# turlando/flac-py

Measured on AMD Instinct MI355X. Metric: PCM samples/sec encode-analysis, 4608-blk/16-bit mono, 1/2/4/8 MI355X, higher is better.
Workload: dtype i16 in; f64 autocorrelation/Levinson; i32 predictors; 1 GPU; 1e6 synthetic mono 4608-sample int16 blocks, -l 12 -q 5 -r 0,5; units_per_gpu=1000000, units_total=1000000, block=4608, sample_bits=16, max_lpc_order=12, qlp_precision=5, mode=reference, parallelism=dp1 (block shards), open_eighths=0, lpc_pruning=on: candidates proven to lose skipped (sign bound, partial-sum tiers)

## Files before the change

### flac-py_amd/abi.py

```python
import ctypes as C

import numpy as np

ABI_VERSION = 6
MAX_LPC_ORDER = 32
MAX_BLOCK = 65535
MAX_RICE_ORDER = 15
STATS_WORDS = 128
E_INVALID, E_HIP, E_UNSUPPORTED, E_NOMEM = -1, -2, -3, -4


def lpc_rec_words(L: int) -> int:
    return 2 + L + (L * (L + 1)) // 2


STATUS_OK = 0
STATUS_ZERO_DIVISION = 1
STATUS_ASSERTION = 2
STATUS_VALUE_ERROR = 3
STATUS_OVERFLOW = 4
STATUS_RESIDUAL_WIDE = 16
STATUS_FRAME_TOO_LARGE = 17
STATUS_EOF = 5
STATUS_VERIFY = 18
# ... 369 lines not shown
                                          C.c_int32, C.c_void_p, C.c_void_p, C.c_void_p, C.c_int64, C.c_int64,
                                          C.POINTER(InfoResult)]),
    "flacmi_stream_stats": (C.c_int, [C.c_void_p, C.c_void_p, C.c_int64, C.c_int32, C.c_int32,
                                      C.c_int64, C.c_void_p, C.c_void_p]),
    "flacmi_comm_available": (C.c_int, []),
    "flacmi_unit_stride": (C.c_int64, [C.c_int32, C.c_int32]),
    "flacmi_comm_id": (C.c_int, [C.c_void_p]),
    "flacmi_comm_init": (C.c_int, [C.c_void_p, C.c_int, C.c_int, C.c_void_p, C.POINTER(C.c_void_p)]),
    "flacmi_allreduce_stats": (C.c_int, [C.c_void_p, C.c_void_p, C.c_void_p]),
    "flacmi_comm_destroy": (C.c_int, [C.c_void_p]),
    "flacmi_synth_device": (C.c_int, [C.c_void_p, C.c_void_p, C.c_int32, C.c_int32, C.c_int64,
                                      C.c_int64, C.c_int64, C.c_int32, C.c_uint64, C.c_void_p]),
    "flacmi_synth_mix_device": (C.c_int, [C.c_void_p, C.c_void_p, C.c_int32, C.c_int32, C.c_int64,
                                          C.c_int64, C.c_int64, C.c_int32, C.c_uint64, C.c_int32, C.c_void_p]),
    "flacmi_device_alloc": (C.c_void_p, [C.c_void_p, C.c_size_t]),
    "flacmi_device_free": (C.c_int, [C.c_void_p, C.c_void_p]),
    "flacmi_memcpy_h2d": (C.c_int, [C.c_void_p, C.c_void_p, C.c_void_p, C.c_size_t]),
    "flacmi_memcpy_d2h": (C.c_int, [C.c_void_p, C.c_void_p, C.c_void_p, C.c_size_t]),
    "flacmi_synchronize": (C.c_int, [C.c_void_p]),
    "flacmi_last_timing": (C.c_int, [C.c_void_p, C.POINTER(C.c_float), C.c_int]),
    "flacmi_timing_reset": (C.c_int, [C.c_void_p]),
    "flacmi_set_knob": (C.c_int, [C.c_char_p, C.c_int32]),
    "flacmi_get_knob": (C.c_int, [C.c_char_p, C.POINTER(C.c_int32)]),
    "flacmi_host_pypow2": (C.c_double, [C.c_double, C.POINTER(C.c_int32)]),
    "flacmi_host_floor_log2": (C.c_int32, [C.c_double]),
    "flacmi_device_selftest": (C.c_int, [C.c_void_p, C.c_int32, C.c_void_p, C.c_void_p, C.c_void_p,
                                         C.c_int64]),
    "flacmi_device_lpc_from_acf": (C.c_int, [C.c_void_p, C.c_void_p, C.c_int64, C.c_int32, C.c_int32,
                                             C.c_void_p]),
}
```

### flac-py_amd/csrc/flacmi_host.cpp

```cpp
#include <dlfcn.h>
#include <hip/hip_runtime.h>

#include <algorithm>
#include <atomic>
#include <cerrno>
#include <chrono>
#include <cmath>
#include <cstdarg>
#include <cstdio>
#include <cstdlib>
#include <cstring>
#include <map>
#include <mutex>
#include <string>
#include <vector>

#include "../../include/flacmi.h"
#include "flacmi_kernels.h"
#include "pymath.h"
#include "device_common.h"

using namespace flacmi;

static double (*volatile libm_cos)(double) = cos;
// ... 102 lines not shown
struct flacmi_ctx {
    int device = 0;
    hipStream_t stream = nullptr;
    double* d_log2thr = nullptr;
    int32_t* d_sintab = nullptr;
    std::map<int, double*> windows;
    std::map<int, std::pair<int, int>> window_one;
    std::map<int, uint16_t*> chunk_weights;
    DevBuf bound;
    DevBuf rec, retry, h_samples, h_meta, h_params, h_residual, h_acf, h_fs, h_ls, h_recs;
    uint16_t* d_crc = nullptr;
    DevBuf scan, h_offsets, h_status, h_frames, dec, slow;
    DevBuf h_subkind;
    DevBuf h_wasted;
    DevBuf h_side, h_choice;
    DevBuf idx, sd_data, sd_table, sd_meta, sd_rows, sd_pcm;
    DevBuf si_frames, si_subs, si_parts;
    int64_t frames_bytes = 0;
    static constexpr int kRing = 64;
    static constexpr int kMaxChunks = 8;
    hipEvent_t ev[kRing][3 + 2 * kMaxChunks] = {};
    int nchunks[kRing] = {};
    hipEvent_t lpc_done[kMaxChunks] = {};
    int ncalls = 0;
    struct EncState* enc = nullptr;
};
static void enc_free(struct EncState* es);
static int enc_streams(flacmi_ctx* ctx);
static hipStream_t enc_side(flacmi_ctx* ctx);

static int ensure_buf(DevBuf& b, size_t bytes) {
    if (b.bytes >= bytes && b.p) return 0;
    if (b.p) HIP_TRY(hipFree(b.p));
    b.p = nullptr;
    b.bytes = 0;
    size_t want = bytes + bytes / 8 + 4096;
    HIP_TRY(hipMalloc(&b.p, want));
    b.bytes = want;
    return 0;
}

static int64_t row_pitch(int64_t n, int64_t sample_bytes) {
    int64_t bytes = ((n * sample_bytes + 15) / 16) * 16;
    if (bytes % 4096 == 0) bytes += 128;
    return bytes / sample_bytes;
}

static int set_device(flacmi_ctx* ctx) {
    if (!ctx) return fail(FLACMI_E_INVALID, "null context");
    HIP_TRY(hipSetDevice(ctx->device));
    return 0;
}

namespace {
struct KnobDef {
    const char* name;
    int dflt;
};
constexpr KnobDef kKnobs[kKnobCount] = {{"FLACMI_OVERLAP", -1}, {"FLACMI_MF8_GRID", 0}, {"FLACMI_STREAM_GENERIC", 0}, {"FLACMI_DECODE_GENERIC", 0},
                                        {"FLACMI_PACK_GENERIC", 0}, {"FLACMI_DECODE_LPC", 1}, {"FLACMI_ENERGY_BOUND", 1}, {"FLACMI_INFO_GRID", 0},
                                        {"FLACMI_RICE_GRID", 0}};
std::atomic<int> g_knob[kKnobCount];
std::once_flag g_knob_once;
void knobs_init() {
    std::call_once(g_knob_once, [] {
        for (int i = 0; i < kKnobCount; ++i) {
            const char* e = getenv(kKnobs[i].name);
            g_knob[i].store(e && e[0] ? atoi(e) : kKnobs[i].dflt);
        }
    });
}
int knob_index(const char* name) {
    if (!name) return -1;
    for (int i = 0; i < kKnobCount; ++i)
        if (strcmp(name, kKnobs[i].name) == 0) return i;
    return -1;
}
}

int flacmi::knob(Knob k) {
    knobs_init();
    return g_knob[k].load(std::memory_order_relaxed);
}

extern "C" {

int flacmi_set_knob(const char* name, int32_t value) {
    const int i = knob_index(name);
    if (i < 0) return fail(FLACMI_E_INVALID, "unknown knob %s", name ? name : "(null)");
    knobs_init();
    g_knob[i].store(value);
    return 0;
}

int flacmi_get_knob(const char* name, int32_t* value) {
    const int i = knob_index(name);
    if (i < 0 || !value) return fail(FLACMI_E_INVALID, "unknown knob %s", name ? name : "(null)");
    *value = knob((Knob)i);
    return 0;
}

int flacmi_abi_version(void) { return FLACMI_ABI_VERSION; }

const char* flacmi_last_error(void) { return g_err.c_str(); }

int flacmi_device_count(void) {
    int n = 0;
    if (hipGetDeviceCount(&n) != hipSuccess) return 0;
    return n;
}

flacmi_ctx* flacmi_create(int device) {
    ensure_tables();
    if (!g_tables_error.empty()) {
        fail(FLACMI_E_UNSUPPORTED, "%s", g_tables_error.c_str());
        return nullptr;
    }
    int ndev = 0;
    if (hipGetDeviceCount(&ndev) != hipSuccess || ndev <= 0) {
        fail(FLACMI_E_HIP, "no HIP device available");
        return nullptr;
    }
    if (device < 0 || device >= ndev) {
        fail(FLACMI_E_INVALID, "device %d out of range (0..%d)", device, ndev - 1);
        return nullptr;
    }
    flacmi_ctx* ctx = new flacmi_ctx();
    ctx->device = device;
    auto bad = [&](hipError_t e, const char* what) {
        fail(FLACMI_E_HIP, "%s: %s", what, hipGetErrorString(e));
        flacmi_destroy(ctx);
        return (flacmi_ctx*)nullptr;
    };
    hipError_t e;
    if ((e = hipSetDevice(device)) != hipSuccess) return bad(e, "hipSetDevice");
    if ((e = hipStreamCreateWithFlags(&ctx->stream, hipStreamNonBlocking)) != hipSuccess) return bad(e, "hipStreamCreate");
    for (auto& slot : ctx->ev)
        for (auto& ev : slot)
            if ((e = hipEventCreate(&ev)) != hipSuccess) return bad(e, "hipEventCreate");
    for (auto& ev : ctx->lpc_done)
        if ((e = hipEventCreateWithFlags(&ev, hipEventDisableTiming)) != hipSuccess) return bad(e, "hipEventCreate");
    if ((e = hipMalloc(&ctx->d_log2thr, sizeof(double) * PYM_LOG2_THR_N)) != hipSuccess) return bad(e, "hipMalloc");
    if ((e = hipMemcpy(ctx->d_log2thr, g_log2thr.data(), sizeof(double) * PYM_LOG2_THR_N, hipMemcpyHostToDevice)) != hipSuccess)
        return bad(e, "hipMemcpy");
    if ((e = hipMalloc(&ctx->d_sintab, sizeof(int32_t) * 4096)) != hipSuccess) return bad(e, "hipMalloc");
    if ((e = hipMemcpy(ctx->d_sintab, g_sintab.data(), sizeof(int32_t) * 4096, hipMemcpyHostToDevice)) != hipSuccess)
        return bad(e, "hipMemcpy");
    const std::vector<uint16_t> crc = crc16_tables();
    if ((e = hipMalloc(&ctx->d_crc, sizeof(uint16_t) * crc.size())) != hipSuccess) return bad(e, "hipMalloc");
    if ((e = hipMemcpy(ctx->d_crc, crc.data(), sizeof(uint16_t) * crc.size(), hipMemcpyHostToDevice)) != hipSuccess)
        return bad(e, "hipMemcpy");
    return ctx;
}

void flacmi_destroy(flacmi_ctx* ctx) {
    if (!ctx) return;
    (void)hipSetDevice(ctx->device);
    (void)hipDeviceSynchronize();
    enc_free(ctx->enc);
    for (auto& kv : ctx->windows) (void)hipFree(kv.second);
    for (auto& kv : ctx->chunk_weights) (void)hipFree(kv.second);
    for (DevBuf* b : {&ctx->bound, &ctx->idx, &ctx->sd_data, &ctx->sd_table, &ctx->sd_meta, &ctx->sd_rows, &ctx->sd_pcm, &ctx->si_frames, &ctx->si_subs, &ctx->si_parts, &ctx->slow, &ctx->dec, &ctx->rec, &ctx->retry, &ctx->h_samples, &ctx->h_meta, &ctx->h_params, &ctx->h_residual, &ctx->h_acf,
                      &ctx->h_fs, &ctx->h_ls, &ctx->h_recs, &ctx->scan, &ctx->h_offsets, &ctx->h_status,
                      &ctx->h_frames, &ctx->h_subkind, &ctx->h_side, &ctx->h_choice, &ctx->h_wasted})
        if (b->p) (void)hipFree(b->p);
    if (ctx->d_log2thr) (void)hipFree(ctx->d_log2thr);
    if (ctx->d_sintab) (void)hipFree(ctx->d_sintab);
    if (ctx->d_crc) (void)hipFree(ctx->d_crc);
    for (auto& slot : ctx->ev)
        for (auto& ev : slot)
            if (ev) (void)hipEventDestroy(ev);
    if (ctx->stream) (void)hipStreamDestroy(ctx->stream);
    for (auto& ev : ctx->lpc_done)
        if (ev) (void)hipEventDestroy(ev);
    delete ctx;
}

}

static void bound_tables(const std::vector<double>& w, int n, double* kappa, std::vector<uint16_t>& cw) {
    for (int k = 1; k <= kBoundLags; ++k) {
        double m = 0.0;
        for (int i = k; i <= n - 2; ++i) m = std::max(m, fabs(w[i] - w[i - k]));
        kappa[k - 1] = m * (1.0 + ldexp(1.0, -50));
    }
    cw.assign((size_t)(n + 7) / 8, 0);
    for (int c = 2; 8 * c < n; ++c) {
        double m = 1.0;
        for (int i = 8 * c; i < 8 * c + 8; ++i) m = std::min(m, i < n - 1 ? w[i] : 0.0);
        cw[c] = (uint16_t)floor(256.0 * m);
    }
}

static int get_window(flacmi_ctx* ctx, int n, double** out, int* one_lo = nullptr, int* one_hi = nullptr,
                      const uint16_t** chunk_weight = nullptr) {
    auto it = ctx->windows.find(n);
    if (it == ctx->windows.end()) {
// ... 165 lines not shown
#ifndef FLACMI_CLASS_LISTS
#define FLACMI_CLASS_LISTS 1
#endif
static int overlap_mode() { return knob(kKnobOverlap); }

static int analyze_device_impl(flacmi_ctx* ctx, const flacmi_batch* b, const flacmi_params* p,
                               const flacmi_outputs* o, hipStream_t s, bool allow_overlap = true) {
    if (int rc = set_device(ctx)) return rc;
    const bool lpc = p->mode == FLACMI_MODE_REFERENCE || p->mode == FLACMI_MODE_LPC_ONLY;
    const int L = lpc ? p->max_lpc_order : 0;
    const int rec_words = FLACMI_LPC_REC_WORDS(L);
    if (lpc) {
        if (int rc = ensure_buf(ctx->rec, sizeof(int32_t) * (size_t)rec_words * (size_t)(b->n_units > 0 ? b->n_units : 1)))
            return rc;
    }
    const int energy = debug_stop() >= 11 ? 0 : knob(kKnobEnergyBound);
    const bool prune_call = p->mode == FLACMI_MODE_REFERENCE && !o->lpc_sums &&
                            !(p->reserved[1] & (FLACMI_FLAG_ALL_CANDIDATES | FLACMI_FLAG_LPC_SIGN | FLACMI_FLAG_SIZE_CHOICE)) && prune_allowed();
    const bool ebound = energy != 0 && prune_call && L >= 1 && L <= 12 && b->sample_bytes == 2 && p->qlp_precision <= 16;
    if (ebound) {
        if (int rc = ensure_buf(ctx->bound, sizeof(uint32_t) * kBoundWords * (size_t)(b->n_units > 0 ? b->n_units : 1))) return rc;
    }
    constexpr int64_t kSubWords = 64 * 16;
    if (int rc = ensure_buf(ctx->retry, sizeof(int64_t) * (size_t)(kSubWords + 2 * b->n_units + 68))) return rc;
    struct Cls {
        int64_t unit0, count;
        int n;
    } cls[2];
    int ncls = 0;
    const int64_t nfull = b->n_units - b->n_tail_units;
    if (b->n_tail_units == 0 || b->tail_len == b->block_len) {
        cls[ncls++] = {0, b->n_units, b->block_len};
    } else {
        if (nfull > 0) cls[ncls++] = {0, nfull, b->block_len};
        cls[ncls++] = {nfull, b->n_tail_units, b->tail_len};
    }
    if (o->acf && !lpc)
        HIP_TRY(hipMemsetAsync(o->acf, 0, sizeof(double) * 33 * b->n_units, s));
    struct Chunk {
        int64_t unit0, count;
        int n;
    } ch[flacmi_ctx::kMaxChunks];
    auto lpc_params_for = [&](int n) {
        LpcArgs a{};
        a.stride = b->unit_stride;
        a.sample_bytes = b->sample_bytes;
        a.n = n;
        a.L = L;
        return a;
    };
    int nch = 0;
    const int ov = lpc ? overlap_mode() : 0;
    const int want = ov > 1 ? ov : 1;
    bool overlap = want > 1 && b->n_units >= 2 * kOverlapMinUnits;
    for (int c = 0; c < ncls; ++c) {
        if (ov < -1 || (ov == -1 && cls[c].count >= 2 * kOverlapMinUnits)) {
            const int64_t R = ov < -1 ? -(int64_t)ov : lpc_units_per_round(lpc_params_for(cls[c].n));
            const int64_t whole = R > 0 ? cls[c].count / R * R : 0, rest = cls[c].count - whole;
            if (whole > 0 && rest > 0 && (ov < -1 || rest >= kOverlapMinUnits) &&
                nch + 2 + (ncls - 1 - c) <= flacmi_ctx::kMaxChunks) {
                ch[nch++] = {cls[c].unit0, whole, cls[c].n};
                ch[nch++] = {cls[c].unit0 + whole, rest, cls[c].n};
                overlap = true;
                continue;
            }
        }
        int64_t k = overlap && ov > 1 ? cls[c].count / kOverlapMinUnits : 1;
        const int left = flacmi_ctx::kMaxChunks - nch - (ncls - 1 - c);
        k = k < 1 ? 1 : k > want ? want : k;
        k = k > left ? left : k;
        for (int64_t i = 0; i < k; ++i) {
            const int64_t u0 = cls[c].count * i / k, u1 = cls[c].count * (i + 1) / k;
            ch[nch++] = {cls[c].unit0 + u0, u1 - u0, cls[c].n};
        }
    }
    auto lpc_args = [&](const Chunk& k, LpcArgs& a) -> int {
        a = LpcArgs{};
        a.samples = b->samples;
        a.stride = b->unit_stride;
        a.unit0 = k.unit0;
        a.count = k.count;
        a.sample_bytes = b->sample_bytes;
        a.n = k.n;
        a.L = L;
        a.q = p->qlp_precision;
        a.lpc_sign = (p->reserved[1] & FLACMI_FLAG_LPC_SIGN) != 0;
        if (int rc = get_window(ctx, k.n, (double**)&a.window, &a.fuse_lo, &a.fuse_hi)) return rc;
        a.bound = ebound ? (uint32_t*)ctx->bound.p + kBoundWords * k.unit0 : nullptr;
        if (b->sample_bits > 26) a.fuse_lo = a.fuse_hi = 0;
        a.log2thr = ctx->d_log2thr;
        a.rec = (int32_t*)ctx->rec.p + k.unit0 * rec_words;
        a.rec_words = rec_words;
        a.acf = o->acf ? o->acf + k.unit0 * 33 : nullptr;
        return 0;
    };
    auto resid_args = [&](const Chunk& k, ResidArgs& a, int& path) -> hipError_t {
// ... 1 lines not shown
        a.samples = b->samples;
        a.stride = b->unit_stride;
        a.unit0 = k.unit0;
        a.count = k.count;
        a.sample_bytes = b->sample_bytes;
        a.n = k.n;
        a.L = L;
        a.mode = p->mode;
        a.rmin = p->rice_min;
        a.rmax = p->rice_max;
        a.rec = lpc ? (const int32_t*)ctx->rec.p + k.unit0 * rec_words : nullptr;
        a.rice_order = p->mode == FLACMI_MODE_RICE_ONLY ? p->reserved[0] : 0;
        a.rec_words = rec_words;
        a.log2thr = ctx->d_log2thr;
        a.meta = o->meta + k.unit0;
        a.rice_params = o->rice_params + k.unit0 * o->params_stride;
        a.params_stride = o->params_stride;
        a.residual = (char*)o->residual + (size_t)k.unit0 * o->residual_stride * o->residual_bytes;
        a.residual_stride = o->residual_stride;
        a.fixed_sums = o->fixed_sums ? o->fixed_sums + k.unit0 * 5 : nullptr;
        a.lpc_sums = o->lpc_sums ? o->lpc_sums + k.unit0 * 32 : nullptr;
        a.stop_after = debug_stop();
        a.mfma = use_mfma();
        int64_t* const rb = (int64_t*)ctx->retry.p;
        a.retry_sub = (unsigned long long*)rb;
        a.retry_count = (unsigned long long*)(rb + kSubWords);
        a.retry_list = rb + kSubWords + 2;
        a.retry2_count = (unsigned long long*)(rb + kSubWords + 2 + b->n_units + 64);
        a.retry2_list = rb + kSubWords + 4 + b->n_units + 64;
        a.sample_bits = b->sample_bits;
        a.stream = use_stream();
        a.prune = prune_call;
        if (ebound) {
            double* w = nullptr;
            if (get_window(ctx, k.n, &w, nullptr, nullptr, &a.chunk_weight)) return hipErrorOutOfMemory;
            a.bound = (const uint32_t*)ctx->bound.p + kBoundWords * k.unit0;
            a.energy = energy;
        }
        a.sign_bound = !(p->reserved[1] & FLACMI_FLAG_TIERS_ONLY) && sign_bound_allowed();
        const bool wide = needs_wide(k.n, b->sample_bits, L, p->qlp_precision, p->mode);
        path = (wide || o->residual_bytes == 8) ? 2 : (b->sample_bytes == 2 && p->qlp_precision <= 16) ? 0 : 1;
        if (path == 2 && o->residual_bytes == 4 && split_ok(b->sample_bits, L, p->qlp_precision)) path = 3;
        return hipSuccess;
    };
    auto launch_resid_chunk = [&](const Chunk& k, hipStream_t st) -> hipError_t {
        ResidArgs a;
        int path = 0;
        if (hipError_t e = resid_args(k, a, path); e != hipSuccess) return e;
        return launch_resid(a, path, o->residual_bytes, st);
    };
    const int slot = ctx->ncalls % flacmi_ctx::kRing;
    hipEvent_t* ev = ctx->ev[slot];
    hipStream_t side = nullptr;
    if (overlap && !allow_overlap) overlap = false;
    if (overlap) {
        if (int rc = enc_streams(ctx)) return rc;
        side = enc_side(ctx);
        if (side == s) overlap = false;
    }
    const bool size_choice = (p->reserved[1] & FLACMI_FLAG_SIZE_CHOICE) != 0;
    if (size_choice) overlap = false;
    ctx->nchunks[slot] = overlap ? nch : 0;
    HIP_TRY(hipEventRecord(ev[0], s));
    if (overlap) {
        HIP_TRY(hipStreamWaitEvent(side, ev[0], 0));
        for (int i = 0; i < nch; ++i) {
            LpcArgs a;
            if (int rc = lpc_args(ch[i], a)) return rc;
            HIP_TRY(launch_lpc(a, side));
            HIP_TRY(hipEventRecord(ctx->lpc_done[i], side));
        }
        HIP_TRY(hipEventRecord(ev[1], side));
        for (int i = 0; i < nch;) {
            int j = i + 1;
            while (j < nch && ch[j].n == ch[i].n && ch[j].unit0 == ch[j - 1].unit0 + ch[j - 1].count) ++j;
            ResidArgs ca;
            int cpath = 0;
            const Chunk whole{ch[i].unit0, ch[j - 1].unit0 + ch[j - 1].count - ch[i].unit0, ch[i].n};
            HIP_TRY(resid_args(whole, ca, cpath));
            const bool merged = FLACMI_CLASS_LISTS && j - i > 1 && stream_class_ok(ca, cpath, o->residual_bytes);
            for (int c = i; c < j; ++c) {
                HIP_TRY(hipStreamWaitEvent(s, ctx->lpc_done[c], 0));
                HIP_TRY(hipEventRecord(ev[3 + 2 * c], s));
                if (merged) {
                    ResidArgs a;
                    int path = 0;
                    HIP_TRY(resid_args(ch[c], a, path));
                    if (c == i) HIP_TRY(launch_stream_class_begin(ca, s));
                    HIP_TRY(launch_stream_class_batch(a, ch[c].unit0 - whole.unit0, whole.count, s));
                    if (c == j - 1) HIP_TRY(launch_stream_class_lists(ca, s));
                } else {
                    HIP_TRY(launch_resid_chunk(ch[c], s));
                }
                HIP_TRY(hipEventRecord(ev[4 + 2 * c], s));
            }
            i = j;
        }
    } else {
        for (int i = 0; i < nch && lpc; ++i) {
            LpcArgs a;
            if (int rc = lpc_args(ch[i], a)) return rc;
            HIP_TRY(launch_lpc(a, s));
        }
        HIP_TRY(hipEventRecord(ev[1], s));
        for (int i = 0; i < nch && !size_choice; ++i) HIP_TRY(launch_resid_chunk(ch[i], s));
    }
    if (size_choice) {
        SizeArgs sa{};
        sa.samples = b->samples;
        sa.stride = b->unit_stride;
        sa.sample_bytes = b->sample_bytes;
        sa.block_len = b->block_len;
        sa.tail_len = b->n_tail_units ? b->tail_len : b->block_len;
        sa.n_units = b->n_units;
        sa.n_tail_units = b->n_tail_units;
        sa.L = L;
        sa.q = p->qlp_precision;
        sa.mode = p->mode;
        sa.rmin = p->rice_min;
        sa.rmax = p->rice_max;
        sa.ss = p->reserved[2] ? p->reserved[2] : b->sample_bits;
        sa.rec = lpc ? (const int32_t*)ctx->rec.p : nullptr;
        sa.rec_words = rec_words;
        sa.meta = o->meta;
        sa.rice_params = o->rice_params;
        sa.params_stride = o->params_stride;
        sa.residual = o->residual;
        sa.residual_stride = o->residual_stride;
// ... 1724 lines not shown
```

### flac-py_amd/csrc/flacmi_kernels.h

```cpp
#pragma once
#include <hip/hip_runtime.h>
#include <stdint.h>

#include "../../include/flacmi.h"

namespace flacmi {

constexpr int kWindowPad = 80;

struct LpcArgs {
    const void* samples;
    int64_t stride;
    int64_t unit0, count;
    int32_t sample_bytes;
    int32_t n, L, q;
    const double* window;
    const double* log2thr;
    int32_t* rec;
    int32_t rec_words;
    int32_t lpc_sign;
    double* acf;
    int32_t fuse_lo, fuse_hi;
    uint32_t* bound;
};
constexpr int kBoundWords = 8;
constexpr uint32_t kBoundUnusable = 0xffffffffu;
constexpr uint32_t kBoundOutside = 0xfffffffeu;
constexpr int kBoundLags = 13;
constexpr int kCoefLimit = 127;

struct ResidArgs {
    const void* samples;
    int64_t stride;
    int64_t unit0, count;
    int32_t sample_bytes;
    int32_t n, L, mode;
    int32_t rmin, rmax;
    int32_t rice_order;
    const int32_t* rec;
    int32_t rec_words;
    const double* log2thr;
    flacmi_unit_meta* meta;
    int32_t* rice_params;
    int64_t params_stride;
    void* residual;
    int64_t residual_stride;
    int64_t* fixed_sums;
    int64_t* lpc_sums;
    int32_t stop_after;
    int32_t mfma;
    unsigned long long* retry_count;
    int64_t* retry_list;
    unsigned long long* retry2_count;
    int64_t* retry2_list;
    unsigned long long* retry_sub;
    int64_t retry_sub_cap;
    int32_t sample_bits;
    int32_t stream;
    int32_t prune;
    int32_t persist;
    int32_t sign_bound;
    const uint32_t* bound;
    const uint16_t* chunk_weight;
    int32_t energy;
    int64_t list_off;
};
#define FLACMI_STATUS_RETRY 0x7e

struct StereoChoice {
    int32_t code;
    int32_t status;
    int64_t unit[2];
};

struct FrameArgs {
    const void* samples;
    int64_t stride;
    int32_t sample_bytes;
    int32_t block_len, tail_len;
    int64_t n_units, n_tail_units;
    int32_t channels, sample_size, q;
    int64_t first_frame, n_frames;
    const flacmi_unit_meta* meta;
    const int32_t* rice_params;
    int64_t params_stride;
    const void* residual;
    int32_t residual_bytes;
    int64_t residual_stride;
// ... 105 lines not shown
    uint8_t* parts;
    int32_t part_stride;
    const uint16_t* crc_slice;
    int32_t wasted_spec;
};

struct PcmArgs {
    const flacmi_pcm_frame* frames;
    int64_t n_frames;
    int32_t channels, bytes_per_sample, raw;
    uint8_t* out;
    int64_t capacity;
    int32_t* status;
};

struct ResidLaunch {
    int threads;
    size_t lds_bytes;
};

ResidLaunch resid_launch_config(int n, int rmax_eff, int residual_bytes);
constexpr int kMaxFinestParts = 4096;

enum Knob { kKnobOverlap = 0, kKnobMf8Grid, kKnobStreamGeneric, kKnobDecodeGeneric, kKnobPackGeneric, kKnobDecodeLpc, kKnobEnergyBound, kKnobInfoGrid, kKnobRiceGrid, kKnobCount };
int knob(Knob k);

hipError_t launch_lpc(const LpcArgs& a, hipStream_t s);
int64_t lpc_units_per_round(const LpcArgs& a);
hipError_t launch_poison_lds(hipStream_t s);
hipError_t launch_export(const int64_t* off, const int32_t* st, int64_t nf, int64_t* h_off, int32_t* h_st,
                         hipStream_t s);
hipError_t launch_lpc_from_acf(const LpcArgs& a, hipStream_t s);
hipError_t launch_resid(const ResidArgs& a, int path, int residual_bytes, hipStream_t s);
bool stream_class_ok(const ResidArgs& cls, int path, int residual_bytes);
hipError_t launch_stream_class_begin(const ResidArgs& cls, hipStream_t s);
hipError_t launch_stream_class_batch(const ResidArgs& chunk, int64_t list_off, int64_t class_count, hipStream_t s);
hipError_t launch_stream_class_lists(const ResidArgs& cls, hipStream_t s);
hipError_t launch_expand_records(const int32_t* rec, int32_t rec_words, int32_t L, int64_t count,
                                 int32_t* out, hipStream_t s);
hipError_t launch_synth(void* dst, int32_t sample_bytes, int32_t bits, int64_t stride,
                        int64_t first_unit, int64_t n_units, int32_t len, uint64_t seed,
                        const int32_t* sintab, int32_t open8, hipStream_t s);
hipError_t launch_stats(const flacmi_unit_meta* meta, int64_t n_units, int32_t block_len,
                        int32_t tail_len, int64_t n_tail_units, int64_t* stats, hipStream_t s);

hipError_t launch_stereo_rows(const void* lr, int32_t sample_bytes, int64_t lr_stride, int64_t n_frames,
                              int32_t block_len, int32_t tail_len, int32_t has_tail, void* mid, int64_t mid_stride,
                              int32_t* side, int64_t side_stride, hipStream_t s);
hipError_t launch_wasted_rows(const void* in, int32_t sample_bytes, int64_t in_stride, int64_t n_units,
                              int32_t block_len, int32_t tail_len, int64_t n_tail_units, int32_t sample_bits,
                              void* out, int64_t out_stride, int32_t* wasted, hipStream_t s);
struct RiceArgs {
    flacmi_unit_meta* meta;
    int32_t* rice_params;
    int64_t params_stride;
    const void* residual;
    int64_t residual_stride;
    int64_t n_units, n_tail_units;
    int32_t block_len, tail_len;
// ... 44 lines not shown
```

### flac-py_amd/csrc/k_lpc.hip

```cpp
#include <type_traits>

#include <map>
#include <mutex>
#include <utility>

#include "device_common.h"

namespace flacmi {


template <int LMAX>
__device__ __forceinline__ void write_quant(int32_t* rec, int L, int p, const int32_t* q, int nq,
                                            int shift) {
    rec[2 + p - 1] = shift;
    int32_t* c = rec + 2 + L + (p * (p - 1)) / 2;
#pragma unroll
    for (int j = 0; j < LMAX; ++j)
        if (j < p) c[j] = j < nq ? q[j] : 0;
}

template <int LMAX, bool EB = false>
__device__ __forceinline__ void lpc_finish(const double (&acc)[LMAX + 1], const LpcArgs& a, int32_t* __restrict__ rec,
                                           uint32_t* __restrict__ bound = nullptr) {
    const int L = a.L, q = a.q;
    const bool eb = EB && bound != nullptr;
    const __attribute__((address_space(4))) double* kap =
        (const __attribute__((address_space(4))) double*)a.window + a.n + kWindowPad - 1;
    double emax = 0.0, u2max = 0.0, samax = 0.0;
    double emax2 = 0.0, u2max2 = 0.0;
    bool ebad = false;
    const pym::PowTables PT{c_log_hdr, c_log_tab, c_exp_hdr, c_exp_tab};
    double c[LMAX + 1];
    c[0] = 1.0;
#pragma unroll
    for (int j = 1; j <= LMAX; ++j) c[j] = 0.0;
    double err = acc[0];
    int lst = ST_OK, lsite = 0, qst = ST_OK, qsite = 0;
    uint32_t negmask = 0;
    const double qmax = (double)((1LL << (q - 1)) - 1);
    const double qmin = -(double)(1LL << (q - 1));
    const uint64_t sign = a.lpc_sign ? 1ull << 63 : 0;
    static_for<LMAX>([&](auto K_) {
        constexpr int k = K_;
        if (k < L && lst == ST_OK) {
            double lam = 0.0;
#pragma unroll
// ... 106 lines not shown
    });
    int st = lst != ST_OK ? lst : qst;
    int site = lst != ST_OK ? lsite : qsite;
    if (st == ST_OK && L == 0) {
        st = ST_VALUE;
        site = FLACMI_SITE_LPC_EMPTY;
    }
    rec[0] = st | (site << 16);
    rec[1] = (int32_t)negmask;
    if constexpr (EB) {
        if (eb) {
            const double u1 = __builtin_ceil(__builtin_sqrt((double)a.n * emax) * (1.0 + 0x1p-40)) + 1.0;
            const double u2 = __builtin_ceil(256.0 * u2max * (1.0 + 0x1p-40)) + 1.0;
            const bool ok = st == ST_OK && negmask == 0 && !ebad && samax <= (double)kCoefLimit && u1 < 4294967295.0 &&
                            u2 < 4294967295.0;
            const bool out = st == ST_OK && samax > (double)kCoefLimit;
            const double v1 = L > 1 ? __builtin_ceil(__builtin_sqrt((double)a.n * emax2) * (1.0 + 0x1p-40)) + 1.0 : 0.0;
            const double v2 = L > 1 ? __builtin_ceil(256.0 * u2max2 * (1.0 + 0x1p-40)) + 1.0 : 0.0;
            const uint32_t w0 = ok ? (uint32_t)u1 : kBoundUnusable, w1 = ok ? (uint32_t)u2 : out ? kBoundOutside : kBoundUnusable;
            const uint32_t w2 = ok ? (uint32_t)v1 : 0u, w3 = ok ? (uint32_t)v2 : 0u;
            const uint32_t w4 = ok ? ((uint32_t)rec[2 + L] & 0xffffu) | (uint32_t)rec[2] << 16 : 0u;
            reinterpret_cast<uint4*>(bound)[0] = uint4{w0, w1, w2, w3};
            reinterpret_cast<uint4*>(bound)[1] = uint4{w4, 0u, 0u, 0u};
        }
    }
}

constexpr int lpc_waves(int lmax, int sample_bytes = 4) { return lmax <= 12 ? 3 : sample_bytes == 4 ? 2 : 1; }

template <int LMAX, typename SampleT, bool ACF_IN = false>
__global__ __launch_bounds__(256) __attribute__((amdgpu_waves_per_eu(lpc_waves(LMAX, (int)sizeof(SampleT))))) void k_lpc(LpcArgs a) {
    const int64_t gid = (int64_t)blockIdx.x * 256 + threadIdx.x;
    if (gid >= a.count) return;
    const int64_t u = a.unit0 + gid;
    const SampleT* __restrict__ x = (const SampleT*)a.samples + u * a.stride;
    int32_t* __restrict__ rec = a.rec + gid * a.rec_words;
    const int n = a.n, L = a.L;

    constexpr int S = ((LMAX + 1 + 7) / 8) * 8;
    double acc[LMAX + 1];
    if constexpr (ACF_IN) {
#pragma unroll
        for (int l = 0; l <= LMAX; ++l) acc[l] = l <= L ? a.acf[gid * 33 + l] : 0.0;
    } else {
    if (n >= 4 && n <= 7) {
        rec[0] = ST_ZERODIV | (FLACMI_SITE_TUKEY << 16);
// ... 131 lines not shown
                for (int t = 0; t < S; ++t) {
                    const double av = (double)sample(cur, sb * S + t) * win[m0 + t];
                    ring[t] = av;
#pragma unroll
                    for (int l = 0; l <= LMAX; ++l) {
                        const double prev = ring[(t - l + S) % S];
                        acc[l] = acc[l] + prev * av;
                    }
                }
            }
        }
#pragma unroll
        for (int w = 0; w < W; ++w) cur[w] = nxt[w];
    }
    }
    if (a.acf) {
        double* o = a.acf + gid * 33;
#pragma unroll
        for (int l = 0; l < 33; ++l) o[l] = (l <= LMAX && l <= L) ? acc[l < LMAX ? l : LMAX] : 0.0;
    }
    }

    constexpr bool EB = !ACF_IN && LMAX <= 12 && sizeof(SampleT) == 2;
    lpc_finish<LMAX, EB>(acc, a, rec, EB && a.bound ? a.bound + kBoundWords * gid : nullptr);
}


template <int LMAX>
__global__ __launch_bounds__(256) __attribute__((amdgpu_waves_per_eu(LMAX <= 12 ? 4 : 1))) void k_lpc_tile(LpcArgs a) {
    __shared__ __align__(16) uint4 tiles[4 * 512];
    const int lane = threadIdx.x & 63, wid = threadIdx.x >> 6;
    const int64_t wave0 = (int64_t)blockIdx.x * 256 + wid * 64;
    if (wave0 >= a.count) return;
    const int64_t gid = wave0 + lane;
    const int n = a.n, L = a.L;
    int32_t* __restrict__ rec = a.rec + gid * a.rec_words;
    constexpr int S = ((LMAX + 1 + 7) / 8) * 8;
    static_assert(32 % S == 0, "ring length divides a half tile");
    static_assert(64 <= kWindowPad, "the last tile's window reads stay inside the window's zero pad");
    double acc[LMAX + 1];
    if (n >= 4 && n <= 7) {
        rec[0] = ST_ZERODIV | (FLACMI_SITE_TUKEY << 16);
        rec[1] = 0;
        if (a.acf)
            for (int l = 0; l < 33; ++l) a.acf[gid * 33 + l] = 0.0;
        return;
    }
// ... 70 lines not shown
                        for (int l = 0; l <= LMAX; ++l) {
                            const double prev = ring[(t - l + S) % S];
                            acc[l] = acc[l] + prev * av;
                        }
                    }
                }
            }
        }
    };
    int t1 = (a.fuse_lo + LMAX + 63) >> 6;
    if (a.fuse_lo + LMAX <= 0) t1 = 0;
    int t2 = min(a.fuse_hi, M) >> 6;
    if (t2 > ntile) t2 = ntile;
    if (t1 > t2) t1 = t2;
    if (ntile > 0) issue(0);
    for (int tI = 0; tI < t1; ++tI) tile_body(tI, T0{});
    for (int tI = t1; tI < t2; ++tI) tile_body(tI, T1{});
    for (int tI = t2; tI < ntile; ++tI) tile_body(tI, T0{});
    if (a.acf) {
        double* o = a.acf + gid * 33;
#pragma unroll
        for (int l = 0; l < 33; ++l) o[l] = (l <= LMAX && l <= L) ? acc[l < LMAX ? l : LMAX] : 0.0;
    }
    lpc_finish<LMAX, (LMAX <= 12)>(acc, a, rec, a.bound ? a.bound + kBoundWords * gid : nullptr);
}


static bool lpc_tile_enabled() {
    static const bool on = [] {
        const char* e = getenv("FLACMI_LPC_TILE");
        return !(e && e[0] == '0');
    }();
    return on;
}

template <int LMAX>
static hipError_t launch_lpc_T(const LpcArgs& a, hipStream_t s) {
    const dim3 grid((unsigned)((a.count + 255) / 256));
    if constexpr (LMAX <= 12) {
        const int64_t full = a.count & ~(int64_t)63;
        if (a.sample_bytes == 2 && lpc_tile_enabled() && a.stride % 8 == 0 && a.stride >= 8 && full > 0) {
            LpcArgs t = a;
            t.count = full;
            hipLaunchKernelGGL((k_lpc_tile<LMAX>), dim3((unsigned)((full + 255) / 256)), dim3(256), 0, s, t);
            if (full == a.count) return hipGetLastError();
            LpcArgs r = a;
            r.unit0 += full;
            r.count = a.count - full;
            r.rec += full * a.rec_words;
            if (r.bound) r.bound += kBoundWords * full;
            if (r.acf) r.acf += full * 33;
            hipLaunchKernelGGL((k_lpc<LMAX, int16_t>), dim3((unsigned)((r.count + 255) / 256)), dim3(256), 0, s, r);
            return hipGetLastError();
        }
    }
    if (a.sample_bytes == 2)
        hipLaunchKernelGGL((k_lpc<LMAX, int16_t>), grid, dim3(256), 0, s, a);
    else
        hipLaunchKernelGGL((k_lpc<LMAX, int32_t>), grid, dim3(256), 0, s, a);
    return hipGetLastError();
}

hipError_t launch_lpc_from_acf(const LpcArgs& a, hipStream_t s) {
    if (a.count <= 0) return hipSuccess;
    hipLaunchKernelGGL((k_lpc<32, int32_t, true>), dim3((unsigned)((a.count + 255) / 256)), dim3(256), 0, s, a);
    return hipGetLastError();
}

template <int LMAX>
static const void* lpc_kernel_T(const LpcArgs& a) {
    if constexpr (LMAX <= 12)
        if (a.sample_bytes == 2 && lpc_tile_enabled() && a.stride % 8 == 0 && a.stride >= 8)
            return reinterpret_cast<const void*>(&k_lpc_tile<LMAX>);
// ... 34 lines not shown
```

### flac-py_amd/csrc/k_stream.hip

```cpp
#include <type_traits>

#include "device_common.h"

namespace flacmi {

namespace {

typedef _Float16 h8 __attribute__((ext_vector_type(8)));
typedef float f4 __attribute__((ext_vector_type(4)));
typedef _Float16 h2 __attribute__((ext_vector_type(2)));
typedef unsigned short us2 __attribute__((ext_vector_type(2)));

#ifndef FLACMI_STREAM_CPT
#define FLACMI_STREAM_CPT 5
#endif
constexpr int kSCPT = FLACMI_STREAM_CPT;
#ifndef FLACMI_RICE_DEDUP
#define FLACMI_RICE_DEDUP 1
#endif
#ifndef FLACMI_SAD16
#define FLACMI_SAD16 1
#endif
#ifndef FLACMI_FIXED_STRIDE8
#define FLACMI_FIXED_STRIDE8 1
// ... 270 lines not shown
        uint4 q[kSCPT];
#pragma unroll
        for (int j = 0; j < kSCPT; ++j) {
#if FLACMI_NT_LOAD
            typedef unsigned int v4u __attribute__((ext_vector_type(4)));
            const v4u t = __builtin_nontemporal_load(reinterpret_cast<const v4u*>(src) + min(tid + j * NT, nch - 1));
            q[j] = uint4{t.x, t.y, t.z, t.w};
#else
            q[j] = src[min(tid + j * NT, nch - 1)];
#endif
        }
        if constexpr (S8) {
            fixb8[0] = reinterpret_cast<const uint4*>(kFixB8a.w)[lane];
            fixb8[1] = reinterpret_cast<const uint4*>(kFixB8b.w)[lane];
        } else {
            fixb = reinterpret_cast<const uint4*>(kFixB.w)[lane];
        }
        if constexpr (EL) {
            st_entry = (int)opaque_s((uint32_t)st_entry);
            bw_entry.x = opaque_s(bw_entry.x);
            bw_entry.y = opaque_s(bw_entry.y);
#pragma unroll
            for (int i = 0; i < 3; ++i) b2_entry[i] = opaque_s(b2_entry[i]);
        }
        uint32_t cwv[EB ? kSCPT : 1];
        if constexpr (EB) {
#pragma unroll
            for (int j = 0; j < kSCPT; ++j) cwv[j] = a.chunk_weight[min(tid + j * NT, nch - 1)];
        }
        int32_t tv[kTJ > 0 ? kTJ : 1][2];
        if constexpr (NG > 0 && !EB) {
            const int32_t* r = a.rec + gid * rw;
#pragma unroll
            for (int j = 0; j < kTJ; ++j) {
                if (j > 0 && j * NT >= kTW) break;
                const int gw = tid + j * NT, p = gw / 10 + 1, w = gw - 10 * (p - 1);
                const int pc = p < L ? p : L, base = 2 + L + (pc * (pc - 1)) / 2;
                tv[j][0] = r[w == 8 ? 1 + pc : min(max(base + 15 - 2 * w, 0), rw - 1)];
                tv[j][1] = r[min(max(base + 14 - 2 * w, 0), rw - 1)];
            }
        }
        if (tid < kSHP) xs[tid - kSHP] = 0x8000u;
        if (tid < Pmax) pks[tid] = a.stop_after == 10 ? (uint32_t)n * 40u : 0u;
#if FLACMI_SAD16
        const uint32_t k8000 = opaque(0x80008000u);
#else
// ... 949 lines not shown
}

static hipError_t launch_stream_G(const ResidArgs& a, bool list, hipStream_t s) {
    if (a.mode == FLACMI_MODE_FIXED_ONLY) return launch_stream_T<0>(a, list, s);
    if (a.L <= 4) return launch_stream_T<1>(a, list, s);
    if (a.L <= 8) return launch_stream_T<2>(a, list, s);
    return launch_stream_T<3>(a, list, s);
}

static hipError_t launch_stream_lists(const ResidArgs& a, hipStream_t s) {
    hipError_t e;
    if ((e = launch_poison_lds(s)) != hipSuccess) return e;
    if ((e = launch_stream_G(a, true, s)) != hipSuccess) return e;
    if ((e = launch_poison_lds(s)) != hipSuccess) return e;
    ResidArgs b = a;
    b.retry_count = a.retry2_count;
    b.retry_list = a.retry2_list;
    return a.L <= 8 ? launch_resid_retry_l8(b, s) : launch_resid_retry_l12(b, s);
}

hipError_t launch_resid_stream(const ResidArgs& a_in, hipStream_t s) {
    ResidArgs a = a_in;
    a.list_off = 0;
    a.retry_sub_cap = (a.count + 63) / 64;
    hipError_t e = hipMemsetAsync(a.retry_sub, 0, 64 * 16 * sizeof(unsigned long long), s);
    if (e != hipSuccess) return e;
    if ((e = launch_stream_G(a, false, s)) != hipSuccess) return e;
    if (a.mode == FLACMI_MODE_FIXED_ONLY) return hipSuccess;
    if ((e = hipMemsetAsync(a.retry2_count, 0, sizeof(unsigned long long), s)) != hipSuccess) return e;
    return launch_stream_lists(a, s);
}

bool stream_class_ok(const ResidArgs& cls, int path, int residual_bytes) {
    return stream_shape_ok(cls, path, residual_bytes) && cls.mode == FLACMI_MODE_REFERENCE && cls.prune && cls.energy != 0 &&
           cls.bound && cls.chunk_weight;
}
hipError_t launch_stream_class_begin(const ResidArgs& cls, hipStream_t s) {
    hipError_t e = hipMemsetAsync(cls.retry_sub, 0, 64 * 16 * sizeof(unsigned long long), s);
    if (e != hipSuccess) return e;
    return hipMemsetAsync(cls.retry2_count, 0, sizeof(unsigned long long), s);
}
hipError_t launch_stream_class_batch(const ResidArgs& chunk, int64_t list_off, int64_t class_count, hipStream_t s) {
    if (chunk.count <= 0) return hipSuccess;
    ResidArgs a = chunk;
    a.list_off = list_off;
    a.retry_sub_cap = (class_count + 63) / 64;
    if (hipError_t e = launch_poison_lds(s); e != hipSuccess) return e;
    return launch_stream_G(a, false, s);
}
hipError_t launch_stream_class_lists(const ResidArgs& cls, hipStream_t s) {
    ResidArgs a = cls;
    a.list_off = 0;
    a.retry_sub_cap = (cls.count + 63) / 64;
    return launch_stream_lists(a, s);
}

}
```

### include/flacmi.h

```cpp
#ifndef FLACMI_H
#define FLACMI_H

#include <stddef.h>
#include <stdint.h>

#ifdef __cplusplus
extern "C" {
#endif

#define FLACMI_ABI_VERSION 6
#define FLACMI_MAX_LPC_ORDER 32
#define FLACMI_MAX_BLOCK 65535
#define FLACMI_MAX_RICE_ORDER 15
#define FLACMI_LPC_REC_WORDS(L) (2 + (L) + ((L) * ((L) + 1)) / 2)

enum flacmi_error {
    FLACMI_OK = 0,
    FLACMI_E_INVALID = -1,
    FLACMI_E_HIP = -2,
    FLACMI_E_UNSUPPORTED = -3,
    FLACMI_E_NOMEM = -4,
};

enum flacmi_status {
// ... 367 lines not shown
int flacmi_allreduce_stats(flacmi_comm* comm, int64_t* d_stats, void* stream);
int flacmi_comm_destroy(flacmi_comm* comm);

int64_t flacmi_unit_stride(int32_t block_len, int32_t sample_bytes);

int flacmi_synth_device(flacmi_ctx* ctx, void* dst, int32_t sample_bytes, int32_t sample_bits,
                        int64_t unit_stride, int64_t first_unit, int64_t n_units, int32_t len,
                        uint64_t seed, void* stream);
int flacmi_synth_mix_device(flacmi_ctx* ctx, void* dst, int32_t sample_bytes, int32_t sample_bits,
                            int64_t unit_stride, int64_t first_unit, int64_t n_units, int32_t len,
                            uint64_t seed, int32_t open_eighths, void* stream);

void* flacmi_device_alloc(flacmi_ctx* ctx, size_t bytes);
int flacmi_device_free(flacmi_ctx* ctx, void* ptr);
int flacmi_memcpy_h2d(flacmi_ctx* ctx, void* dst, const void* src, size_t bytes);
int flacmi_memcpy_d2h(flacmi_ctx* ctx, void* dst, const void* src, size_t bytes);
int flacmi_synchronize(flacmi_ctx* ctx);

int flacmi_last_timing(flacmi_ctx* ctx, float* ms, int n);
int flacmi_timing_reset(flacmi_ctx* ctx);

int flacmi_set_knob(const char* name, int32_t value);
int flacmi_get_knob(const char* name, int32_t* value);

double flacmi_host_pypow2(double x, int32_t* status);
int32_t flacmi_host_floor_log2(double x);

int flacmi_device_selftest(flacmi_ctx* ctx, int32_t which, const double* x, double* out,
                           int32_t* status, int64_t n);
int flacmi_device_lpc_from_acf(flacmi_ctx* ctx, const double* acf, int64_t n, int32_t L, int32_t q,
                               int32_t* rec);

#ifdef __cplusplus
}
#endif
#endif
```

Baseline: 463.2 billion samples/s.

## Build LPC retry lists in the LPC kernel and run list pass on side stream

The LPC kernel now appends units whose energy bound is unusable to per-class retry lists via atomics. The stream kernel skips those units early, and the list-processing pass is launched on the side stream right after LPC, overlapping the residual batches. Retry buffers are doubled, one region per class, so both groups can build lists independently. This adds atomics in the LPC finish path and a cross-stream dependency, and it includes a debug count-readout API.

```diff
diff --git a/flac-py_amd/abi.py b/flac-py_amd/abi.py
--- a/flac-py_amd/abi.py
+++ b/flac-py_amd/abi.py
@@ -415,6 +415,7 @@
     "flacmi_timing_reset": (C.c_int, [C.c_void_p]),
     "flacmi_set_knob": (C.c_int, [C.c_char_p, C.c_int32]),
     "flacmi_get_knob": (C.c_int, [C.c_char_p, C.POINTER(C.c_int32)]),
+    "flacmi_debug_list_counts": (C.c_int, [C.c_void_p, C.c_int32, C.POINTER(C.c_uint64)]),
     "flacmi_host_pypow2": (C.c_double, [C.c_double, C.POINTER(C.c_int32)]),
     "flacmi_host_floor_log2": (C.c_int32, [C.c_double]),
     "flacmi_device_selftest": (C.c_int, [C.c_void_p, C.c_int32, C.c_void_p, C.c_void_p, C.c_void_p,
diff --git a/flac-py_amd/csrc/flacmi_host.cpp b/flac-py_amd/csrc/flacmi_host.cpp
--- a/flac-py_amd/csrc/flacmi_host.cpp
+++ b/flac-py_amd/csrc/flacmi_host.cpp
@@ -148,6 +148,8 @@
     hipEvent_t ev[kRing][3 + 2 * kMaxChunks] = {};
     int nchunks[kRing] = {};
     hipEvent_t lpc_done[kMaxChunks] = {};
+    hipEvent_t lists_done = nullptr;
+    int64_t retry_words = 0, retry2_off = 0;
     int ncalls = 0;
     struct EncState* enc = nullptr;
 };
@@ -185,7 +187,7 @@
 };
 constexpr KnobDef kKnobs[kKnobCount] = {{"FLACMI_OVERLAP", -1}, {"FLACMI_MF8_GRID", 0}, {"FLACMI_STREAM_GENERIC", 0}, {"FLACMI_DECODE_GENERIC", 0},
                                         {"FLACMI_PACK_GENERIC", 0}, {"FLACMI_DECODE_LPC", 1}, {"FLACMI_ENERGY_BOUND", 1}, {"FLACMI_INFO_GRID", 0},
-                                        {"FLACMI_RICE_GRID", 0}};
+                                        {"FLACMI_RICE_GRID", 0}, {"FLACMI_LPC_LISTS", 1}};
 std::atomic<int> g_knob[kKnobCount];
 std::once_flag g_knob_once;
 void knobs_init() {
@@ -223,6 +225,19 @@
     const int i = knob_index(name);
     if (i < 0 || !value) return fail(FLACMI_E_INVALID, "unknown knob %s", name ? name : "(null)");
     *value = knob((Knob)i);
+    return 0;
+}
+
+int flacmi_debug_list_counts(flacmi_ctx* ctx, int32_t cls, uint64_t* counts) {
+    if (!ctx || !counts || cls < 0 || cls > 1) return fail(FLACMI_E_INVALID, "bad argument");
+    if (!ctx->retry.p || ctx->retry_words == 0) return fail(FLACMI_E_INVALID, "no analysis call yet");
+    if (int rc = set_device(ctx)) return rc;
+    HIP_TRY(hipDeviceSynchronize());
+    const int64_t* rb = (const int64_t*)ctx->retry.p + ctx->retry_words * cls;
+    std::vector<uint64_t> sub(64 * 16);
+    HIP_TRY(hipMemcpy(sub.data(), rb, sizeof(uint64_t) * sub.size(), hipMemcpyDeviceToHost));
+    for (int r = 0; r < 64; ++r) counts[r] = sub[16 * r];
+    HIP_TRY(hipMemcpy(&counts[64], rb + ctx->retry2_off, sizeof(uint64_t), hipMemcpyDeviceToHost));
     return 0;
 }
 
@@ -266,6 +281,7 @@
             if ((e = hipEventCreate(&ev)) != hipSuccess) return bad(e, "hipEventCreate");
     for (auto& ev : ctx->lpc_done)
         if ((e = hipEventCreateWithFlags(&ev, hipEventDisableTiming)) != hipSuccess) return bad(e, "hipEventCreate");
+    if ((e = hipEventCreateWithFlags(&ctx->lists_done, hipEventDisableTiming)) != hipSuccess) return bad(e, "hipEventCreate");
     if ((e = hipMalloc(&ctx->d_log2thr, sizeof(double) * PYM_LOG2_THR_N)) != hipSuccess) return bad(e, "hipMalloc");
     if ((e = hipMemcpy(ctx->d_log2thr, g_log2thr.data(), sizeof(double) * PYM_LOG2_THR_N, hipMemcpyHostToDevice)) != hipSuccess)
         return bad(e, "hipMemcpy");
@@ -299,6 +315,7 @@
     if (ctx->stream) (void)hipStreamDestroy(ctx->stream);
     for (auto& ev : ctx->lpc_done)
         if (ev) (void)hipEventDestroy(ev);
+    if (ctx->lists_done) (void)hipEventDestroy(ctx->lists_done);
     delete ctx;
 }
 
@@ -510,7 +527,10 @@
         if (int rc = ensure_buf(ctx->bound, sizeof(uint32_t) * kBoundWords * (size_t)(b->n_units > 0 ? b->n_units : 1))) return rc;
     }
     constexpr int64_t kSubWords = 64 * 16;
-    if (int rc = ensure_buf(ctx->retry, sizeof(int64_t) * (size_t)(kSubWords + 2 * b->n_units + 68))) return rc;
+    const int64_t retry_words = kSubWords + 2 * b->n_units + 68;
+    if (int rc = ensure_buf(ctx->retry, sizeof(int64_t) * (size_t)retry_words * 2)) return rc;
+    ctx->retry_words = retry_words;
+    ctx->retry2_off = kSubWords + 2 + b->n_units + 64;
     struct Cls {
         int64_t unit0, count;
         int n;
@@ -528,6 +548,7 @@
     struct Chunk {
         int64_t unit0, count;
         int n;
+        int cls;
     } ch[flacmi_ctx::kMaxChunks];
     auto lpc_params_for = [&](int n) {
         LpcArgs a{};
@@ -547,8 +568,8 @@
             const int64_t whole = R > 0 ? cls[c].count / R * R : 0, rest = cls[c].count - whole;
             if (whole > 0 && rest > 0 && (ov < -1 || rest >= kOverlapMinUnits) &&
                 nch + 2 + (ncls - 1 - c) <= flacmi_ctx::kMaxChunks) {
-                ch[nch++] = {cls[c].unit0, whole, cls[c].n};
-                ch[nch++] = {cls[c].unit0 + whole, rest, cls[c].n};
+                ch[nch++] = {cls[c].unit0, whole, cls[c].n, c};
+                ch[nch++] = {cls[c].unit0 + whole, rest, cls[c].n, c};
                 overlap = true;
                 continue;
             }
@@ -559,7 +580,7 @@
         k = k > left ? left : k;
         for (int64_t i = 0; i < k; ++i) {
             const int64_t u0 = cls[c].count * i / k, u1 = cls[c].count * (i + 1) / k;
-            ch[nch++] = {cls[c].unit0 + u0, u1 - u0, cls[c].n};
+            ch[nch++] = {cls[c].unit0 + u0, u1 - u0, cls[c].n, c};
         }
     }
     auto lpc_args = [&](const Chunk& k, LpcArgs& a) -> int {
@@ -607,7 +628,7 @@
         a.lpc_sums = o->lpc_sums ? o->lpc_sums + k.unit0 * 32 : nullptr;
         a.stop_after = debug_stop();
         a.mfma = use_mfma();
-        int64_t* const rb = (int64_t*)ctx->retry.p;
+        int64_t* const rb = (int64_t*)ctx->retry.p + retry_words * k.cls;
         a.retry_sub = (unsigned long long*)rb;
         a.retry_count = (unsigned long long*)(rb + kSubWords);
         a.retry_list = rb + kSubWords + 2;
@@ -646,49 +667,104 @@
     const bool size_choice = (p->reserved[1] & FLACMI_FLAG_SIZE_CHOICE) != 0;
     if (size_choice) overlap = false;
     ctx->nchunks[slot] = overlap ? nch : 0;
+    struct Group {
+        int i, j;
+        Chunk whole;
+        ResidArgs ca;
+        int cpath;
+        bool lpc_lists;
+    } grp[2];
+    int ngrp = 0;
+    for (int i = 0; i < nch && ngrp < 2;) {
+        int j = i + 1;
+        while (j < nch && ch[j].cls == ch[i].cls) ++j;
+        Group& g = grp[ngrp++];
+        g.i = i;
+        g.j = j;
+        g.whole = Chunk{ch[i].unit0, ch[j - 1].unit0 + ch[j - 1].count - ch[i].unit0, ch[i].n, ch[i].cls};
+        g.cpath = 0;
+        HIP_TRY(resid_args(g.whole, g.ca, g.cpath));
+        g.lpc_lists = knob(kKnobLpcLists) != 0 && lpc && ebound && !size_choice && g.whole.count > 0 &&
+                      stream_class_ok(g.ca, g.cpath, o->residual_bytes);
+        i = j;
+    }
+    auto lpc_args_in = [&](const Group& g, int c, LpcArgs& a) -> int {
+        if (int rc = lpc_args(ch[c], a)) return rc;
+        if (g.lpc_lists) {
+            a.retry_sub = g.ca.retry_sub;
+            a.retry_list = g.ca.retry_list;
+            a.retry_sub_cap = (g.whole.count + 63) / 64;
+            a.list_off = ch[c].unit0 - g.whole.unit0;
+        }
+        return 0;
+    };
+    auto launch_batch_in = [&](const Group& g, int c, hipStream_t st) -> hipError_t {
+        ResidArgs a;
+        int path = 0;
+        if (hipError_t e = resid_args(ch[c], a, path); e != hipSuccess) return e;
+        return launch_stream_class_batch(a, ch[c].unit0 - g.whole.unit0, g.whole.count, true, st);
+    };
     HIP_TRY(hipEventRecord(ev[0], s));
     if (overlap) {
         HIP_TRY(hipStreamWaitEvent(side, ev[0], 0));
-        for (int i = 0; i < nch; ++i) {
-            LpcArgs a;
-            if (int rc = lpc_args(ch[i], a)) return rc;
-            HIP_TRY(launch_lpc(a, side));
-            HIP_TRY(hipEventRecord(ctx->lpc_done[i], side));
-        }
+        bool side_lists = false;
+        for (int k = 0; k < ngrp; ++k)
+            if (grp[k].lpc_lists) HIP_TRY(launch_stream_class_begin(grp[k].ca, side));
+        for (int k = 0; k < ngrp; ++k)
+            for (int i = grp[k].i; i < grp[k].j; ++i) {
+                LpcArgs a;
+                if (int rc = lpc_args_in(grp[k], i, a)) return rc;
+                HIP_TRY(launch_lpc(a, side));
+                HIP_TRY(hipEventRecord(ctx->lpc_done[i], side));
+            }
         HIP_TRY(hipEventRecord(ev[1], side));
-        for (int i = 0; i < nch;) {
-            int j = i + 1;
-            while (j < nch && ch[j].n == ch[i].n && ch[j].unit0 == ch[j - 1].unit0 + ch[j - 1].count) ++j;
-            ResidArgs ca;
-            int cpath = 0;
-            const Chunk whole{ch[i].unit0, ch[j - 1].unit0 + ch[j - 1].count - ch[i].unit0, ch[i].n};
-            HIP_TRY(resid_args(whole, ca, cpath));
-            const bool merged = FLACMI_CLASS_LISTS && j - i > 1 && stream_class_ok(ca, cpath, o->residual_bytes);
-            for (int c = i; c < j; ++c) {
+        for (int k = 0; k < ngrp; ++k)
+            if (grp[k].lpc_lists) {
+                HIP_TRY(launch_stream_class_lists(grp[k].ca, side));
+                side_lists = true;
+            }
+        if (side_lists) HIP_TRY(hipEventRecord(ctx->lists_done, side));
+        for (int k = 0; k < ngrp; ++k) {
+            const Group& g = grp[k];
+            const bool merged = FLACMI_CLASS_LISTS && !g.lpc_lists && g.j - g.i > 1 && stream_class_ok(g.ca, g.cpath, o->residual_bytes);
+            for (int c = g.i; c < g.j; ++c) {
                 HIP_TRY(hipStreamWaitEvent(s, ctx->lpc_done[c], 0));
                 HIP_TRY(hipEventRecord(ev[3 + 2 * c], s));
-                if (merged) {
+                if (g.lpc_lists) {
+                    HIP_TRY(launch_batch_in(g, c, s));
+                } else if (merged) {
                     ResidArgs a;
                     int path = 0;
                     HIP_TRY(resid_args(ch[c], a, path));
-                    if (c == i) HIP_TRY(launch_stream_class_begin(ca, s));
-                    HIP_TRY(launch_stream_class_batch(a, ch[c].unit0 - whole.unit0, whole.count, s));
-                    if (c == j - 1) HIP_TRY(launch_stream_class_lists(ca, s));
+                    if (c == g.i) HIP_TRY(launch_stream_class_begin(g.ca, s));
+                    HIP_TRY(launch_stream_class_batch(a, ch[c].unit0 - g.whole.unit0, g.whole.count, false, s));
+                    if (c == g.j - 1) HIP_TRY(launch_stream_class_lists(g.ca, s));
                 } else {
                     HIP_TRY(launch_resid_chunk(ch[c], s));
                 }
                 HIP_TRY(hipEventRecord(ev[4 + 2 * c], s));
             }
-            i = j;
-        }
+        }
+        if (side_lists) HIP_TRY(hipStreamWaitEvent(s, ctx->lists_done, 0));
     } else {
-        for (int i = 0; i < nch && lpc; ++i) {
-            LpcArgs a;
-            if (int rc = lpc_args(ch[i], a)) return rc;
-            HIP_TRY(launch_lpc(a, s));
-        }
+        for (int k = 0; k < ngrp; ++k)
+            if (grp[k].lpc_lists) HIP_TRY(launch_stream_class_begin(grp[k].ca, s));
+        for (int k = 0; k < ngrp && lpc; ++k)
+            for (int i = grp[k].i; i < grp[k].j; ++i) {
+                LpcArgs a;
+                if (int rc = lpc_args_in(grp[k], i, a)) return rc;
+                HIP_TRY(launch_lpc(a, s));
+            }
         HIP_TRY(hipEventRecord(ev[1], s));
-        for (int i = 0; i < nch && !size_choice; ++i) HIP_TRY(launch_resid_chunk(ch[i], s));
+        for (int k = 0; k < ngrp && !size_choice; ++k) {
+            if (grp[k].lpc_lists) HIP_TRY(launch_stream_class_lists(grp[k].ca, s));
+            for (int c = grp[k].i; c < grp[k].j; ++c) {
+                if (grp[k].lpc_lists)
+                    HIP_TRY(launch_batch_in(grp[k], c, s));
+                else
+                    HIP_TRY(launch_resid_chunk(ch[c], s));
+            }
+        }
     }
     if (size_choice) {
         SizeArgs sa{};
diff --git a/flac-py_amd/csrc/flacmi_kernels.h b/flac-py_amd/csrc/flacmi_kernels.h
--- a/flac-py_amd/csrc/flacmi_kernels.h
+++ b/flac-py_amd/csrc/flacmi_kernels.h
@@ -22,6 +22,10 @@
     double* acf;
     int32_t fuse_lo, fuse_hi;
     uint32_t* bound;
+    unsigned long long* retry_sub;
+    int64_t* retry_list;
+    int64_t retry_sub_cap;
+    int64_t list_off;
 };
 constexpr int kBoundWords = 8;
 constexpr uint32_t kBoundUnusable = 0xffffffffu;
@@ -64,6 +68,7 @@
     const uint16_t* chunk_weight;
     int32_t energy;
     int64_t list_off;
+    int32_t lpc_lists;
 };
 #define FLACMI_STATUS_RETRY 0x7e
 
@@ -215,7 +220,7 @@
 ResidLaunch resid_launch_config(int n, int rmax_eff, int residual_bytes);
 constexpr int kMaxFinestParts = 4096;
 
-enum Knob { kKnobOverlap = 0, kKnobMf8Grid, kKnobStreamGeneric, kKnobDecodeGeneric, kKnobPackGeneric, kKnobDecodeLpc, kKnobEnergyBound, kKnobInfoGrid, kKnobRiceGrid, kKnobCount };
+enum Knob { kKnobOverlap = 0, kKnobMf8Grid, kKnobStreamGeneric, kKnobDecodeGeneric, kKnobPackGeneric, kKnobDecodeLpc, kKnobEnergyBound, kKnobInfoGrid, kKnobRiceGrid, kKnobLpcLists, kKnobCount };
 int knob(Knob k);
 
 hipError_t launch_lpc(const LpcArgs& a, hipStream_t s);
@@ -227,7 +232,7 @@
 hipError_t launch_resid(const ResidArgs& a, int path, int residual_bytes, hipStream_t s);
 bool stream_class_ok(const ResidArgs& cls, int path, int residual_bytes);
 hipError_t launch_stream_class_begin(const ResidArgs& cls, hipStream_t s);
-hipError_t launch_stream_class_batch(const ResidArgs& chunk, int64_t list_off, int64_t class_count, hipStream_t s);
+hipError_t launch_stream_class_batch(const ResidArgs& chunk, int64_t list_off, int64_t class_count, bool lpc_lists, hipStream_t s);
 hipError_t launch_stream_class_lists(const ResidArgs& cls, hipStream_t s);
 hipError_t launch_expand_records(const int32_t* rec, int32_t rec_words, int32_t L, int64_t count,
                                  int32_t* out, hipStream_t s);
diff --git a/flac-py_amd/csrc/k_lpc.hip b/flac-py_amd/csrc/k_lpc.hip
--- a/flac-py_amd/csrc/k_lpc.hip
+++ b/flac-py_amd/csrc/k_lpc.hip
@@ -21,7 +21,7 @@
 
 template <int LMAX, bool EB = false>
 __device__ __forceinline__ void lpc_finish(const double (&acc)[LMAX + 1], const LpcArgs& a, int32_t* __restrict__ rec,
-                                           uint32_t* __restrict__ bound = nullptr) {
+                                           uint32_t* __restrict__ bound = nullptr, int64_t gid = 0) {
     const int L = a.L, q = a.q;
     const bool eb = EB && bound != nullptr;
     const __attribute__((address_space(4))) double* kap =
@@ -174,6 +174,12 @@
             const uint32_t w4 = ok ? ((uint32_t)rec[2 + L] & 0xffffu) | (uint32_t)rec[2] << 16 : 0u;
             reinterpret_cast<uint4*>(bound)[0] = uint4{w0, w1, w2, w3};
             reinterpret_cast<uint4*>(bound)[1] = uint4{w4, 0u, 0u, 0u};
+            if (a.retry_sub && out) {
+                const int64_t id = gid + a.list_off;
+                const int r = (int)(id & 63);
+                const unsigned long long k = atomicAdd(a.retry_sub + 16 * r, 1ull);
+                a.retry_list[r * a.retry_sub_cap + (int64_t)k] = id;
+            }
         }
     }
 }
@@ -351,7 +357,7 @@
     }
 
     constexpr bool EB = !ACF_IN && LMAX <= 12 && sizeof(SampleT) == 2;
-    lpc_finish<LMAX, EB>(acc, a, rec, EB && a.bound ? a.bound + kBoundWords * gid : nullptr);
+    lpc_finish<LMAX, EB>(acc, a, rec, EB && a.bound ? a.bound + kBoundWords * gid : nullptr, gid);
 }
 
 
@@ -468,7 +474,7 @@
 #pragma unroll
         for (int l = 0; l < 33; ++l) o[l] = (l <= LMAX && l <= L) ? acc[l < LMAX ? l : LMAX] : 0.0;
     }
-    lpc_finish<LMAX, (LMAX <= 12)>(acc, a, rec, a.bound ? a.bound + kBoundWords * gid : nullptr);
+    lpc_finish<LMAX, (LMAX <= 12)>(acc, a, rec, a.bound ? a.bound + kBoundWords * gid : nullptr, gid);
 }
 
 
@@ -495,6 +501,7 @@
             r.count = a.count - full;
             r.rec += full * a.rec_words;
             if (r.bound) r.bound += kBoundWords * full;
+            r.list_off += full;
             if (r.acf) r.acf += full * 33;
             hipLaunchKernelGGL((k_lpc<LMAX, int16_t>), dim3((unsigned)((r.count + 255) / 256)), dim3(256), 0, s, r);
             return hipGetLastError();
diff --git a/flac-py_amd/csrc/k_stream.hip b/flac-py_amd/csrc/k_stream.hip
--- a/flac-py_amd/csrc/k_stream.hip
+++ b/flac-py_amd/csrc/k_stream.hip
@@ -316,6 +316,12 @@
             bw_entry.y = opaque_s(bw_entry.y);
 #pragma unroll
             for (int i = 0; i < 3; ++i) b2_entry[i] = opaque_s(b2_entry[i]);
+        }
+        if constexpr (EB) {
+            if (a.lpc_lists) {
+                const uint2 be = EL ? bw_entry : *reinterpret_cast<const uint2*>(a.bound + kBoundWords * gid);
+                if (be.x == kBoundUnusable && be.y == kBoundOutside) return;
+            }
         }
         uint32_t cwv[EB ? kSCPT : 1];
         if constexpr (EB) {
@@ -1311,6 +1317,7 @@
 hipError_t launch_resid_stream(const ResidArgs& a_in, hipStream_t s) {
     ResidArgs a = a_in;
     a.list_off = 0;
+    a.lpc_lists = 0;
     a.retry_sub_cap = (a.count + 63) / 64;
     hipError_t e = hipMemsetAsync(a.retry_sub, 0, 64 * 16 * sizeof(unsigned long long), s);
     if (e != hipSuccess) return e;
@@ -1329,10 +1336,11 @@
     if (e != hipSuccess) return e;
     return hipMemsetAsync(cls.retry2_count, 0, sizeof(unsigned long long), s);
 }
-hipError_t launch_stream_class_batch(const ResidArgs& chunk, int64_t list_off, int64_t class_count, hipStream_t s) {
+hipError_t launch_stream_class_batch(const ResidArgs& chunk, int64_t list_off, int64_t class_count, bool lpc_lists, hipStream_t s) {
     if (chunk.count <= 0) return hipSuccess;
     ResidArgs a = chunk;
     a.list_off = list_off;
+    a.lpc_lists = lpc_lists ? 1 : 0;
     a.retry_sub_cap = (class_count + 63) / 64;
     if (hipError_t e = launch_poison_lds(s); e != hipSuccess) return e;
     return launch_stream_G(a, false, s);
diff --git a/include/flacmi.h b/include/flacmi.h
--- a/include/flacmi.h
+++ b/include/flacmi.h
@@ -413,6 +413,7 @@
 
 int flacmi_set_knob(const char* name, int32_t value);
 int flacmi_get_knob(const char* name, int32_t* value);
+int flacmi_debug_list_counts(flacmi_ctx* ctx, int32_t cls, uint64_t* counts);
 
 double flacmi_host_pypow2(double x, int32_t* status);
 int32_t flacmi_host_floor_log2(double x);
```

New measurement: 465.2 billion samples/s (median of 6 runs). About the same (+0.4%).
